# DeNA/Chainer_Realtime_Multi-Person_Pose_Estimation

Measured on AMD Instinct MI355X. Metric: frames/sec at 368x368 batch (1/2/4/8 GPU) + keypoint-match vs reference, higher is better.
Workload: dtype f32; 1 GPU; batch32_368x368_synthetic_uint8_per_gpu; per_gpu_batch=32, global_batch=32, map=320x320, weights=seeded He + calibrated head, records_gathered=32, status_bits=0

## Files before the change

### chainer_realtime_multi-person_pose_estimation_amd/csrc/conv_select.hip

```cpp
#include "pmx_common.h"

#include <math.h>
#include <algorithm>
#include <map>
#include <mutex>
#include <tuple>
#include <vector>

bool wino_eligible(int ks, int cin_pad, int cout_pad) { return (ks == 3 || ks == 7) && cin_pad % 32 == 0 && cout_pad % 128 == 0; }

static const double WINO_T7_CHUNK_US = 50.0, WINO_T3_CHUNK_US = 9.3, WINO_PHASE_US = 4.0, WINO_UNIT_FIXED_US = 8.0;

static double wino_tail_makespan(int ks, int nch, int g, long long nblk, int ncu)
{
    std::vector<double> unit_us;
    for (int c = 0; c < nch; c += g) unit_us.push_back(std::min(g, nch - c) * (ks == 7 ? 8.0 : 2.0) * WINO_PHASE_US + WINO_UNIT_FIXED_US);
    if (ks == 7) {
        unit_us.push_back(nch * 2.0 * WINO_PHASE_US + WINO_UNIT_FIXED_US);
        unit_us.push_back(nch * 2.0 * WINO_PHASE_US + WINO_UNIT_FIXED_US);
        unit_us.push_back(nch * 0.5 * WINO_PHASE_US + WINO_UNIT_FIXED_US);
    }
    std::vector<double> cu((size_t)ncu, 0.0);
    auto cmp = [](double a, double b) { return a > b; };
    double end = 0.0;
// ... 85 lines not shown
        const double cost = (double)main_rounds + (best + 10.0) / t_block;
        if (best_g && (o.wino_tail == 1 || cost < plain_cost)) { plain_cost = cost; tg = best_g; }
    }
    if (g) {
        const double t_block = nch * (ks == 7 ? 52e-6 : 18.5e-6);
        const double eff = o.wino_unit_eff / 100.0 * (ks == 7 ? 1.0 : 0.75);
        const long long ublocks = (long long)((H + 7) / 8) * ((W + 15) / 16) * images * nb;
        const double est_unit = (double)ublocks / (ncu * eff) +
                                (double)ublocks * (S + 1) * 65536.0 / 3.0e12 / t_block + 0.03;
        if (est_unit < plain_cost && ublocks * S * 2 >= ncu) { *unit_g = gu; return 2; }
    }
    if (blocks * 100 >= (long long)o.wino_min_fill * rounds * ncu) { *run = geom_run; *tail_g = tg; return 1; }
    return 0;
}

int wino_split_images(const WinoSelectOpts& o, int ks, int cin_pad, int cout_pad, int cout, int ldc, int B, int groups, int H, int W, int pool)
{
    if (!o.wino_split || B < 2 || o.conv_algo != 1) return 0;
    int ug = 0, run = 0, tg = 0;
    if (wino_select(o, ks, cin_pad, cout_pad, cout, ldc, B * groups, H, W, pool, &ug, &run, &tg) != 1) return 0;
    const int nch = cin_pad / 32;
    const long long ncu = o.ncu, nb = cout_pad / 128;
    const long long rects = (long long)((H + 7) / 8) * ((W + 15) / 16);
    long long bpi;
    if (run) {
        const int ntiles = PMX_WINO_RUN_TX * ((H + 1) / 2), nblk = (ntiles + PMX_WINO_RUN_TILES - 1) / PMX_WINO_RUN_TILES, nfull = ntiles / PMX_WINO_RUN_TILES;
        bpi = (long long)(tg ? nfull : nblk) * (W / (PMX_WINO_RUN_TX * 2)) * nb * groups;
    } else
        bpi = rects * nb * groups;
    const long long total = bpi * B, full = total / ncu;
// ... 22 lines not shown
```

### chainer_realtime_multi-person_pose_estimation_amd/csrc/pmx_api.hip

```cpp
#include "pmx_ctx.h"

#include <math.h>
#include <stdarg.h>
#include <stdio.h>
#include <string.h>
#include <algorithm>
#include <functional>
#include <map>

static thread_local char g_err[1024] = "";
void pmx_set_error(const char* fmt, ...)
{
    va_list ap;
    va_start(ap, fmt);
    vsnprintf(g_err, sizeof(g_err), fmt, ap);
    va_end(ap);
}
extern "C" const char* pmx_last_error(void) { return g_err; }
extern "C" const char* pmx_version(void) { return "pose_mi355x 0.1 (gfx950, fp32 MFMA)"; }

extern "C" int pmx_device_count(int* n)
{
    PMX_CHECK(n, PMX_ERR_INVALID, "pmx_device_count: null");
    int c = 0;
// ... 259 lines not shown
    }
    return PMX_OK;
}

extern "C" int pmx_synchronize(pmx_ctx* c)
{
    PMX_CHECK(c, PMX_ERR_INVALID, "null ctx");
    PMX_DEV(c);
    PMX_HIP(hipStreamSynchronize(c->stream));
    return PMX_OK;
}

extern "C" int pmx_set_option(pmx_ctx* c, const char* key, int value)
{
    PMX_CHECK(c && key, PMX_ERR_INVALID, "null arg");
    if (!strcmp(key, "force_variant_k7")) c->opt_force[7] = value;
    else if (!strcmp(key, "force_variant_k3")) c->opt_force[3] = value;
    else if (!strcmp(key, "force_variant_k1")) c->opt_force[1] = value;
    else if (!strcmp(key, "keep_smoothed")) c->opt_keep_smoothed = value;
    else if (!strcmp(key, "stop_stage")) c->opt_stop_stage = value;
    else if (!strcmp(key, "kernel_gen")) c->opt_kernel_gen = value;
    else if (!strcmp(key, "fuse_pairs")) c->opt_fuse_pairs = value;
    else if (!strcmp(key, "fuse_conv1")) c->opt_fuse_conv1 = value;
    else if (!strcmp(key, "conv1_wino")) c->opt_conv1_wino = value;
    else if (!strcmp(key, "precise_lanes")) c->opt_precise_lanes = value < 1 ? 1 : (value > PMX_PR_LANES ? PMX_PR_LANES : value);
    else if (!strcmp(key, "precise_plain")) c->opt_precise_plain = value;
    else if (!strcmp(key, "precise_lane_priority")) c->opt_precise_lane_priority = value != 0;
    else if (!strcmp(key, "precise_table_cap")) c->opt_precise_table_cap = value < 1 ? 1 : value;
    else if (!strcmp(key, "cubic_rows")) c->opt_cubic_rows = value;
    else if (!strcmp(key, "precision")) {
// ... 5 lines not shown
    }
    else if (!strcmp(key, "f16_bn")) {
        PMX_CHECK(value == 0 || value == 64 || value == 128, PMX_ERR_INVALID,
                  "pmx_set_option: \"f16_bn\" = %d: 0 (the launch-size rule), 64 or 128 output channels per block", value);
        c->opt_f16_bn = value;
    }
    else if (!strcmp(key, "conv_algo")) c->opt_conv_algo = value;
    else if (!strcmp(key, "wino_min_fill")) c->opt_wino_min_fill = value;
    else if (!strcmp(key, "wino_unit_eff")) c->opt_wino_unit_eff = value;
    else if (!strcmp(key, "wino_geom")) c->opt_wino_geom = value;
    else if (!strcmp(key, "wino_tail")) c->opt_wino_tail = value;
    else if (!strcmp(key, "wino_tail_g")) c->opt_wino_tail_g = value;
    else if (!strcmp(key, "wino_unit_g")) c->opt_wino_unit_g = value;
    else if (!strcmp(key, "wino_split")) c->opt_wino_split = value;
    else if (!strcmp(key, "wino_tail_merge")) c->opt_wino_tail_merge = value;
    else if (!strcmp(key, "ksplit")) c->opt_ksplit = value;
    else if (!strcmp(key, "ksplit_plan")) c->opt_ksplit = value > 0 ? -value : 0;
    else if (!strcmp(key, "conv_min_lds")) c->opt_conv_min_lds = value;
    else if (!strcmp(key, "conv_v5_lds")) c->opt_conv_v5_lds = value;
    else if (!strcmp(key, "pp_generic")) c->opt_pp_generic = value;
    else if (!strcmp(key, "pp_limbs_slices")) c->opt_limbs_slices = value;
    else if (!strcmp(key, "peaks_gpu_branch")) { c->opt_gpu_branch_peaks = value; c->tab_in_h = -1; }
    else if (!strcmp(key, "kp_flip_x")) c->opt_kp_flip_x = value != 0;
    else if (!strcmp(key, "wgrad_strips")) c->opt_wgrad_strips = value;
    else if (!strcmp(key, "trunk_keep_g")) c->opt_trunk_keep_g = value != 0;
    else { pmx_set_error("pmx_set_option: unknown key '%s'", key); return PMX_ERR_INVALID; }
    return PMX_OK;
}

extern "C" int pmx_set_layer(pmx_ctx* c, const char* name, const float* w, const float* bias, int cout, int cin, int ks)
// ... 42 lines not shown
    DevBuf<T> d;
    int rc;
    if ((rc = d.alloc(j.total))) return rc;
    j.dst = d.get();
    if ((rc = pmx_pack_launch_one(kind, j, st))) return rc;
    PMX_HIP(hipStreamSynchronize(st));
    slot = std::move(d);
    return PMX_OK;
}
static int ensure_wino_pack(hipStream_t st, PackedLayer& L) { return derive_on_device(st, L, PMX_PACK_WINO, L.d_ww, pmx_pack_job_wino(L, nullptr)); }
static int ensure_conv1_pack(hipStream_t st, PackedLayer& L) { return derive_on_device(st, L, PMX_PACK_CONV1, L.d_ww, pmx_pack_job_conv1(L, nullptr)); }
static int ensure_bf16x3_pack(hipStream_t st, PackedLayer& L) { return derive_on_device(st, L, PMX_PACK_BF16X3, L.d_w3, pmx_pack_job_bf16x3(L, nullptr)); }
static int ensure_f16_pack(hipStream_t st, PackedLayer& L) { return derive_on_device(st, L, PMX_PACK_F16, L.d_w16, pmx_pack_job_f16(L, nullptr)); }

static const int SK_ZERO_BIAS = PMX_SK_ZERO_BIAS;
static int sk_reserve(pmx_ctx* c, const FwdCall& k, size_t need)
{
    int rc;
    if ((rc = k.ws.sk_scratch.ensure(need, k.stream))) return rc;
    if (!c->sk_zero_bias) {
        if ((rc = c->sk_zero_bias.alloc(SK_ZERO_BIAS))) return rc;
        PMX_HIP(hipMemsetAsync(c->sk_zero_bias, 0, SK_ZERO_BIAS * sizeof(float), k.stream));
    }
    return PMX_OK;
}
template <typename Reduce>
static int slab_redirect(pmx_ctx* c, const FwdCall& k, const ConvArgs& a0, int groups, int S, size_t slab, unsigned long long kbounds, ConvArgs& a, Reduce& r)
{
    PMX_CHECK(a0.cout_pad <= SK_ZERO_BIAS, PMX_ERR_INVALID, "split-K: cout_pad %d too large", a0.cout_pad);
    if (int rc = sk_reserve(c, k, slab * S * groups)) return rc;
    memset(&r, 0, sizeof r);
    for (int g = 0; g < groups; ++g) {
        float* base = k.ws.sk_scratch + (size_t)g * S * slab;
        r.slabs[g] = base; r.bias[g] = a0.g[g].bias; r.out[g] = a0.g[g].out; r.cout[g] = a0.g[g].cout;
        a.g[g].out = base; a.g[g].bias = c->sk_zero_bias; a.g[g].cout = a0.cout_pad;
    }
    a.ldc = a0.cout_pad; a.relu = 0; a.pool = 0; a.ksplit = S; a.slab_stride = (long long)slab; a.kbounds = kbounds;
    r.slab_stride = (long long)slab; r.B = a0.B; r.H = a0.H; r.W = a0.W; r.ld_slab = a0.cout_pad; r.ldc = a0.ldc;
    r.relu = a0.relu; r.pool = a0.pool;
    return PMX_OK;
}
static int launch_conv(pmx_ctx* c, const FwdCall& k, const ConvArgs& a0, int groups, int v, const SplitPlan& plan)
{
    ConvArgs a = a0;
    if (plan.S <= 1) {
        a.ksplit = 1; a.slab_stride = 0;
        return conv_launch(v, a, groups, c->opt_conv_min_lds, c->opt_conv_v5_lds, k.stream);
    }
    SplitKReduceArgs r;
    int rc = slab_redirect(c, k, a0, groups, plan.S, (size_t)a0.B * a0.H * a0.W * a0.cout_pad, plan.bounds, a, r);
// ... 180 lines not shown
{
    const ConvProf* pf = p.prof ? &p.pf : nullptr;
    if (p.form == FORM_WINO_RUN) return launch_wino_run(c, k, p.a, p.ks, p.groups, p.tail_g, pf);
    int rc;
    if (pf && (rc = prof_begin(c, k, pf->label(), pf->flops, pf->bytes, pf->issued))) return rc;
    switch (p.form) {
    case FORM_F16: rc = conv_f16_launch(p.ks, p.a, p.groups, c->opt_f16_bn, c->num_cus, k.stream); break;
    case FORM_WINO_UNITS: rc = launch_wino_units(c, k, p.a, p.ks, p.groups, p.unit_g); break;
    case FORM_WINO: rc = conv_wino_launch(p.a, p.ks, p.groups, k.stream); break;
    default: rc = launch_conv(c, k, p.a, p.groups, p.variant, p.split); break;
    }
    if (rc) return rc;
    return pf ? prof_end(c, k) : PMX_OK;
}

static int run_conv(pmx_ctx* c, const FwdCall& k, const char* label, PackedLayer* L0, PackedLayer* L1, const float* in0, const float* in1, int lda,
                    float* out0, float* out1, int ldc, int B, int H, int W, int relu, int pool, int level = -1, const char* half = nullptr)
{
    const bool seg = k.seg && level >= 0;
    int rc;
    if (!seg && !half && c->opt_wino_split && B >= 2 && L0->ks > 1 && c->opt_precision != 2 && wino_layers_ok(L0, L1)) {
        const int n0 = wino_split_images(wino_opts(c, k, L0->ks, L1 ? 2 : 1, lda), L0->ks, L0->cin_pad, L0->cout_pad, L0->cout, ldc, B, L1 ? 2 : 1, H, W, pool);
        if (n0 > 0 && n0 < B) {
            const size_t pin = (size_t)n0 * H * W * lda, pout = (size_t)n0 * (pool ? H / 2 : H) * (pool ? W / 2 : W) * ldc;
            const std::string h0 = "@0+" + std::to_string(n0), h1 = "@" + std::to_string(n0) + "+" + std::to_string(B - n0);
            if ((rc = run_conv(c, k, label, L0, L1, in0, in1, lda, out0, out1, ldc, n0, H, W, relu, pool, level, h0.c_str()))) return rc;
            return run_conv(c, k, label, L0, L1, in0 + pin, in1 ? in1 + pin : nullptr, lda, out0 + pout, out1 ? out1 + pout : nullptr, ldc, B - n0, H, W, relu, pool, level,
                            h1.c_str());
        }
    }
    ConvPlan p;
    if ((rc = plan_conv(c, k, p, label, L0, L1, in0, in1, lda, out0, out1, ldc, B, H, W, relu, pool, level))) return rc;
    if (half && p.prof) p.pf.suffix = half;
    return launch_plan(c, k, p);
}

static int run_pair(pmx_ctx* c, const FwdCall& k, const char* labelA, const char* labelB, PackedLayer* a0, PackedLayer* a1, PackedLayer* b0, PackedLayer* b1,
                    const float* in0, const float* in1, int lda, float* mid0, float* mid1, int ldm, float* out0, float* out1, int ldc, int B,
                    int H, int W, int reluB, int level = -1, bool keep_mid = false)
{
    const PackedLayer& LA = *a0;
    const PackedLayer& LB = *b0;
    const int groups = a1 ? 2 : 1;
    const bool seg = k.seg && level >= 0;
    const long long npix = seg ? k.seg->pix[level] : (long long)B * H * W;
    const bool ok = !keep_mid && c->opt_fuse_pairs && c->opt_kernel_gen >= 6 && LA.ks == 1 && LB.ks == 1 && LA.cin_pad == 128 && LB.cin == LA.cout &&
                    conv_pair_supported(LA.cin, LA.cout, LB.cout_pad) && (groups == 1 || b1->cout_pad == LB.cout_pad);
    int rc;
    PMX_CHECK(ok || !seg, PMX_ERR_INVALID, "heterogeneous forward: the 1x1 pair %s + %s has no fused form", labelA, labelB);
    if (!ok) {
        if ((rc = run_conv(c, k, labelA, a0, a1, in0, in1, lda, mid0, mid1, ldm, B, H, W, 1, 0))) return rc;
        return run_conv(c, k, labelB, b0, b1, mid0, mid1, ldm, out0, out1, ldc, B, H, W, reluB, 0);
    }
    PairArgs p;
    memset(&p, 0, sizeof p);
    double flops = 0;
    for (int g = 0; g < groups; ++g) {
        const PackedLayer& A = *(g ? a1 : a0);
        const PackedLayer& Bl = *(g ? b1 : b0);
        p.g[g].in = g ? in1 : in0; p.g[g].w1 = A.d_w; p.g[g].b1 = A.d_b; p.g[g].w2 = Bl.d_w; p.g[g].b2 = Bl.d_b;
        p.g[g].out = g ? out1 : out0; p.g[g].cout = Bl.cout;
        flops += 2.0 * (double)npix * ((double)A.cout * A.cin + (double)Bl.cout * Bl.cin);
    }
    p.npix = npix; p.lda = lda; p.ldc = ldc; p.cmid = LA.cout; p.cout_pad = LB.cout_pad; p.relu2 = reluB;
    if (c->prof_on == 1) {
        const std::string kn = "conv1x1_pair_c" + std::to_string(LA.cout) + "_n" + std::to_string(LB.cout_pad);
        if ((rc = prof_begin(c, k, std::string(labelA) + "+" + labelB + "|" + kn, flops, 4.0 * (double)npix * groups * (LA.cin + LB.cout)))) return rc;
    }
    if ((rc = conv_pair_launch(p, groups, k.stream))) return rc;
    return prof_end(c, k);
}

static bool conv1_pairable(const pmx_ctx* c)
{
    const PackedLayer& L1 = c->layers[c->index.at("conv1_1")];
    const PackedLayer& L2 = c->layers[c->index.at("conv1_2")];
    return c->opt_precision == 0 && c->opt_force[3] < 0 && L1.cin == 3 && L1.cout == 64 && L2.cin == 64 && L2.cout == 64;
}
static bool trunk_retaining(const pmx_ctx* c, const FwdCall& k)
{
    return c->bw.on == 2 && c->kind == NET_POSE && c->ls_on && c->lg_on && c->opt_precision == 0 && !k.seg;
}
static bool conv1_form(const pmx_ctx* c, const FwdCall& k, int B, int H, int W, bool* fuse_out)
// ... 27 lines not shown
    if (seg && c->opt_precision == 2) {
        PMX_CHECK(!in_u8, PMX_ERR_STATE, "conv1: a uint8 input in f16 mode");
        if ((rc = run_conv(c, k, "conv1_1", &L1, nullptr, ws.in16, nullptr, PMX_IN_C, ws.act0, nullptr, 64, B, H, W, 1, 0, 0))) return rc;
        return run_conv(c, k, "conv1_2", &L2, nullptr, ws.act0, nullptr, 64, ws.act1, nullptr, 64, B, H, W, 1, 1, 0);
    }
    PMX_CHECK(!seg || (wino1 && in_u8), PMX_ERR_INVALID, "heterogeneous forward: needs conv1 as conv1_wino_kernel on a uint8 input");
    if (!fuse && !wino1) {
        if ((rc = run_conv(c, k, "conv1_1", &L1, nullptr, ws.in16, nullptr, PMX_IN_C, ws.act0, nullptr, 64, B, H, W, 1, 0))) return rc;
        return run_conv(c, k, "conv1_2", &L2, nullptr, ws.act0, nullptr, 64, ws.act1, nullptr, 64, B, H, W, 1, 1);
    }
    ConvArgs a;
    memset(&a, 0, sizeof a);
    a.g[0].in = ws.in16; a.g[0].w = L2.d_w; a.g[0].bias = L2.d_b; a.g[0].out = ws.act1; a.g[0].cout = L2.cout;
    a.g[1].w = L1.d_w; a.g[1].bias = L1.d_b;
    a.B = B; a.H = H; a.W = W; a.lda = PMX_IN_C; a.ldc = 64; a.nch = L2.nch; a.cout_pad = L2.cout_pad; a.relu = 1; a.pool = 1;
    if (wino1) {
        if ((rc = ensure_wino_pack(k.stream, L2)) || (rc = ensure_conv1_pack(k.stream, L1))) return rc;
        a.g[0].w = L2.d_ww;
        a.g[1].w = L1.d_ww;
        if (in_u8) {
            a.g[1].in = reinterpret_cast<const float*>(in_u8);
            a.kbounds = (unsigned long long)__builtin_bit_cast(unsigned, k.in_div);
        }
        if (seg) { a.nseg = (int)k.seg->segs.size(); a.segs = k.seg->table(PMX_SEG_CONV1); a.seg_tiles = k.seg->tiles[PMX_SEG_CONV1]; }
        if (c->prof_on == 1) {
            const double np0 = seg ? (double)k.seg->pix[0] : (double)B * H * W;
            const double f1 = 2.0 * np0 * 9.0 * (double)L1.cout * L1.cin, f2 = 2.0 * np0 * 9.0 * (double)L2.cout * L2.cin;
            if ((rc = prof_begin(c, k, "conv1_1+conv1_2|conv_wino1_f2x2_t16x16", f1 + f2, (in_u8 ? 3.0 : 4.0 * 3) * np0 + 4.0 * np0 * (64 / 4), f1 + f2 * 16.0 / 36.0))) return rc;
        }
        if ((rc = conv1_wino_launch(a, k.stream))) return rc;
// ... 94 lines not shown
}

int pmx_forward_from_in16(pmx_ctx* c, const FwdCall& k, int B, int H, int W)
{
    PMX_CHECK(!k.seg || c->kind == NET_POSE, PMX_ERR_INVALID, "heterogeneous forward: posenet only");
    if (c->kind != NET_POSE) return forward_cpm(c, k, B, H, W);
    NetBufs& ws = k.ws;
    auto L = [&](const char* n) { return &c->layers[c->index.at(n)]; };
    int rc;
    const int H8 = H / 8, W8 = W / 8;
#define RUN(...) do { if ((rc = run_conv(c, k, __VA_ARGS__))) return rc; } while (0)
    const bool hook = c->ls_on && !k.seg;
    PMX_CHECK(!hook || (&ws == static_cast<NetBufs*>(c) && k.stream == c->stream), PMX_ERR_STATE, "forward: the validation-loss hook covers the context's own working set only");
    BwState& bw = c->bw;
    const bool keep = bw.on && hook && c->lg_on && c->opt_precision == 0;
    bw.valid = bw.done = bw.trunk_done = false;
    const long long npix8 = (long long)B * H8 * W8;
    PMX_CHECK(!keep || (size_t)npix8 <= bw.cap_px, PMX_ERR_CAPACITY, "forward: %lld map pixels, the backward store holds %zu", npix8, bw.cap_px);
    auto slot = [&](int sl, float* else_) { return keep ? bw.act + bw.slot[sl].a_off : else_; };
    float* const x42 = slot(PMX_BW_X42, ws.act1);
    float* const a43 = slot(PMX_BW_C43, ws.act0);
    auto keep_stage = [&](int sl) {
        return keep ? bwd_copy_cols_launch(ws.cat + PMX_CAT_PAF, PMX_CAT_C, bw.act + bw.slot[sl].a_off, 64, npix8, 64, k.stream) : PMX_OK;
    };
    if ((rc = keep && bw.on == 2 ? run_stem_retaining(c, k, B, H, W, x42) : run_stem(c, k, B, H, W, keep ? x42 : nullptr))) return rc;
    RUN("conv4_3_CPM", L("conv4_3_CPM"), nullptr, x42, nullptr, 512, a43, nullptr, 256, B, H8, W8, 1, 0, 3);
    RUN("conv4_4_CPM", L("conv4_4_CPM"), nullptr, a43, nullptr, 256, ws.cat + PMX_CAT_FEAT, nullptr, PMX_CAT_C, B, H8, W8, 1, 0, 3);
    float* cat = ws.cat;
    float* const s51 = slot(PMX_BW_S1 + 0, ws.brA);
    float* const s52 = slot(PMX_BW_S1 + 1, ws.brB);
// ... 21 lines not shown
            in = o;
        }
        snprintf(n1, sizeof n1, "Mconv6_stage%d_L1", s); snprintf(n2, sizeof n2, "Mconv6_stage%d_L2", s);
        snprintf(m1, sizeof m1, "Mconv7_stage%d_L1", s); snprintf(m2, sizeof m2, "Mconv7_stage%d_L2", s);
        snprintf(lab, sizeof lab, "Mconv6_stage%d", s); snprintf(lab2, sizeof lab2, "Mconv7_stage%d", s);
        float* const m6 = slot(PMX_BW_M(s, 6), ws.brB);
        if ((rc = run_pair(c, k, lab, lab2, L(n1), L(n2), L(m1), L(m2), in, in + 128, 256, m6, m6 + 128, 256,
                           cat + PMX_CAT_PAF, cat + PMX_CAT_HEAT, PMX_CAT_C, B, H8, W8, 0, 3, keep))) return rc;
        n_stages = s;
        if (hook && (rc = pmx_loss_stage(c, s, B, H8, W8))) return rc;
        if ((rc = keep_stage(PMX_BW_M(s, 7)))) return rc;
    }
    if (hook && (rc = pmx_loss_finish(c, n_stages, B, H8, W8))) return rc;
    if (keep) { bw.valid = true; bw.stages = n_stages; bw.B = B; bw.fh = H8; bw.fw = W8; bw.t_H = H; bw.t_W = W; }
#undef RUN
    c->maps_valid = true; c->maps_external = false;
    c->cur_B = B; c->cur_fh = H8; c->cur_fw = W8;
    c->cur_segs.clear();
    c->pp_valid = false;
    return PMX_OK;
}

int pmx_check_weights(pmx_ctx* c)
{
    int missing = 0;
    for (auto& l : c->layers) missing += l.set ? 0 : 1;
    PMX_CHECK(missing == 0, PMX_ERR_WEIGHTS, "forward: %d of %d layers have no weights", missing, (int)c->layers.size());
    return PMX_OK;
}
static int check_forward_args(pmx_ctx* c, const void* p, int B, int H, int W)
// ... 24 lines not shown
{
    int rc;
    if (k.seg && c->opt_precision == 2) {
        const long long np0 = k.seg->pix[0];
        PMX_CHECK(np0 >= 1 && np0 <= (long long)c->max_batch * c->max_h * c->max_w && np0 < (1ll << 31), PMX_ERR_CAPACITY,
                  "heterogeneous forward: %lld input pixels", np0);
        if (c->prof_on == 1 && (rc = prof_begin(c, k, "prep_u8|prep_u8", 0, (double)np0 * (3 + 64)))) return rc;
        if ((rc = launch_prep_u8(d, k.ws.in16, 1, 1, (int)np0, divisor, k.stream))) return rc;
        if ((rc = prof_end(c, k))) return rc;
        return pmx_forward_from_in16(c, k, B, H, W);
    }
    if (k.seg || conv1_form(c, k, B, H, W, nullptr)) {
        FwdCall ku = k;
        ku.in_u8 = d; ku.in_div = divisor;
        return pmx_forward_from_in16(c, ku, B, H, W);
    }
    if (c->prof_on == 1 && (rc = prof_begin(c, k, "prep_u8|prep_u8", 0, (double)B * H * W * (3 + 64)))) return rc;
    if ((rc = launch_prep_u8(d, k.ws.in16, B, H, W, divisor, k.stream))) return rc;
    if ((rc = prof_end(c, k))) return rc;
    return pmx_forward_from_in16(c, k, B, H, W);
}

extern "C" int pmx_forward_f32(pmx_ctx* c, const float* x, int B, int H, int W, int on_device)
{
    int rc = check_forward_args(c, x, B, H, W);
    if (rc) return rc;
    PMX_DEV(c);
    const float* d = x;
    if (!on_device) {
        PMX_HIP(hipMemcpyAsync(c->nchw_tmp, x, (size_t)B * H * W * 3 * sizeof(float), hipMemcpyHostToDevice, c->stream));
// ... 313 lines not shown
    PMX_HIP(hipStreamSynchronize(c->stream));
    c->pp_valid = false;
    return pp_realloc(c, cap_pk, cap_sub, candidates, cap_ppl);
}

extern "C" int pmx_get_capacities(pmx_ctx* c, int* peaks_per_joint, int* subsets, int* people, int* candidates)
{
    PMX_CHECK(c, PMX_ERR_INVALID, "null ctx");
    if (peaks_per_joint) *peaks_per_joint = c->pp.cap_pk;
    if (subsets) *subsets = c->pp.cap_sub;
    if (people) *people = c->pp.cap_ppl;
    if (candidates) *candidates = c->pp.cap_cand;
    return PMX_OK;
}

extern "C" int pmx_detect_batch(pmx_ctx* c, const uint8_t* img, int B, int H, int W, int on_device, int map_h, int map_w,
                                double img_len, const double* scale_xy)
{
    int rc = pmx_forward_u8(c, img, B, H, W, on_device);
    if (rc) return rc;
    return pmx_postprocess(c, B, map_h, map_w, img_len, scale_xy);
}

extern "C" int pmx_results_layout(pmx_ctx* c, int* people_cap, size_t* bytes_per_record)
{
    PMX_CHECK(c, PMX_ERR_INVALID, "null ctx");
    PMX_CHECK(c->pp_valid, PMX_ERR_STATE, "pmx_results_layout: no post-process results yet");
    PMX_DEV(c);
    int rc = pp_finalize(c);
    if (rc) return rc;
    if (people_cap) *people_cap = c->pp.cap_ppl;
    if (bytes_per_record) *bytes_per_record = c->pp.rec_bytes;
    return PMX_OK;
// ... 463 lines not shown
```

### chainer_realtime_multi-person_pose_estimation_amd/csrc/pmx_common.h

```cpp
#pragma once
#include <hip/hip_runtime.h>
#include <stdint.h>
#include <stddef.h>
#include <atomic>
#include <string>
#include <vector>

#include "../../include/pose_mi355x.h"
#include "pp_tables.h"

#define PMX_HEATMAP_PEAK_THRESH 0.05f
#define PMX_N_INTEG_POINTS 10
#define PMX_N_INTEG_POINTS_THRESH 8
#define PMX_INNER_PRODUCT_THRESH 0.05
#define PMX_LIMB_LENGTH_RATIO 1.0
#define PMX_LENGTH_PENALTY_VALUE 1.0
#define PMX_N_SUBSET_LIMBS_THRESH 3.0
#define PMX_SUBSET_SCORE_THRESH 0.2
#define PMX_GAUSS_SIGMA 2.5

static const int PMX_LIMBS[PMX_N_LIMBS][2] = {
    {1, 8}, {8, 9}, {9, 10}, {1, 11}, {11, 12}, {12, 13}, {1, 2}, {2, 3}, {3, 4}, {2, 16},
    {1, 5}, {5, 6}, {6, 7}, {5, 17}, {1, 0}, {0, 14}, {0, 15}, {14, 16}, {15, 17}};

// ... 86 lines not shown
int conv_wino_run_launch(const ConvArgs& a, int ks, int groups, hipStream_t stream, hipEvent_t e0 = nullptr, hipEvent_t e1 = nullptr);
int conv_wino_merged_tail_launch(const ConvArgs& a, int ks, int groups, hipStream_t stream);
struct WinoSelectOpts {
    int conv_algo, precision, forced_variant, ksplit, wino_unit_eff, wino_min_fill, wino_geom, wino_tail, wino_tail_g;
    int wino_tail_merge = 1;
    int wino_split = 1;
    int wino_unit_g = 0;
    int groups = 1;
    int lda = 0;
    int ncu;
};
bool wino_eligible(int ks, int cin_pad, int cout_pad);
int wino_select(const WinoSelectOpts& o, int ks, int cin_pad, int cout_pad, int cout, int ldc, int images, int H, int W, int pool, int* unit_g,
                int* run, int* tail_g);
int wino_split_images(const WinoSelectOpts& o, int ks, int cin_pad, int cout_pad, int cout, int ldc, int B, int groups, int H, int W, int pool);
struct SplitPlan { int S; unsigned long long bounds; int sizes[8]; };
struct SplitKReduceArgs {
    const float* slabs[2];
    const float* bias[2];
    float* out[2];
    int cout[2];
    long long slab_stride;
    int ksplit, B, H, W, ld_slab, ldc, relu, pool;
};
int conv_splitk_reduce(const SplitKReduceArgs& r, int groups, hipStream_t stream);
struct PairGroupArgs {
    const float* in;
    const float* w1; const float* b1;
    const float* w2; const float* b2;
    float* out;
// ... 88 lines not shown
```

### chainer_realtime_multi-person_pose_estimation_amd/csrc/pmx_ctx.h

```cpp
#pragma once
#include "pmx_common.h"
#include "pack_index.h"

#include <map>
#include <tuple>
#include <string>
#include <utility>
#include <vector>

template <typename T, bool Host = false>
struct DevBuf {
    T* p = nullptr;
    size_t cap = 0;
    DevBuf() = default;
    DevBuf(const DevBuf&) = delete;
    DevBuf& operator=(const DevBuf&) = delete;
    DevBuf(DevBuf&& o) noexcept { swap(o); }
    DevBuf& operator=(DevBuf&& o) noexcept { reset(); swap(o); return *this; }
    ~DevBuf() { reset(); }
    void swap(DevBuf& o) noexcept { std::swap(p, o.p); std::swap(cap, o.cap); }
    T* get() const { return p; }
    operator T*() const { return p; }
    size_t capacity() const { return cap; }
    void reset()
// ... 121 lines not shown
};

struct SegDesc { int n, H, W; };
enum { PMX_SEG_CONV1 = 0, PMX_SEG_L1 = 1, PMX_SEG_L1P = 2, PMX_SEG_L2 = 3, PMX_SEG_L2P = 4, PMX_SEG_L3 = 5, PMX_SEG_L0 = 6, PMX_SEG_L0P = 7,
       PMX_SEG_TABLES = 8 };
#define PMX_SEG_RECT(level, pool) ((level) == 0 ? ((pool) ? PMX_SEG_L0P : PMX_SEG_L0) : (level) == 1 ? ((pool) ? PMX_SEG_L1P : PMX_SEG_L1) \
                                   : (level) == 2 ? ((pool) ? PMX_SEG_L2P : PMX_SEG_L2) : PMX_SEG_L3)
struct SegGeo { int n, H, W, mh, mw; };
struct SegTables {
    std::vector<SegDesc> segs;
    int tiles[PMX_SEG_TABLES] = {};
    long long pix[4] = {};
    const ConvSeg* dev = nullptr;
    const ConvSeg* table(int t) const { return dev + (size_t)t * segs.size(); }
};
struct FwdCall {
    NetBufs& ws;
    hipStream_t stream;
    int conv_algo;
    const SegTables* seg = nullptr;
    const uint8_t* in_u8 = nullptr;
    float in_div = 255.0f;
};
struct PPCall { PPMaps maps; PPTables tab; int base, B, map_h, map_w; double img_len; bool has_scale; int limbs_slices; };

enum { PMX_BW_C43 = 0, PMX_BW_C44 = 1, PMX_BW_S1 = 2, PMX_BW_M2 = 7, PMX_BW_X42 = 42, PMX_BW_SLOTS = 43 };
#define PMX_BW_M(s, i) (PMX_BW_M2 + ((s) - 2) * 7 + (i) - 1)
struct BwSlot { size_t a_off = 0, g_off = 0; int lda = 0, ldg = 0; };
struct BwState {
    int on = 0;
    bool valid = false;
    bool done = false;
    int stages = 0, B = 0, fh = 0, fw = 0;
    size_t cap_px = 0;
    BwSlot slot[PMX_BW_SLOTS];
    DevBuf<float> act, g;
    DevBuf<float> grad;
// ... 97 lines not shown
    int opt_force[8] = {-1, -1, -1, -1, -1, -1, -1, -1};
    int opt_gpu_branch_peaks = 0;
    int opt_limbs_slices = -1;
    int pp_limbs_slices = 0;
    int opt_kp_flip_x = 0;
    int tab_flip = 0;
    int opt_keep_smoothed = 0, opt_stop_stage = 6, opt_kernel_gen = 6;
    int opt_conv_algo = 1;
    int opt_wino_unit_eff = 80;
    int opt_wino_min_fill = 50;
    int opt_wino_geom = -1;
    int opt_wino_tail = -1;
    int opt_wino_tail_merge = 1;
    int opt_wino_tail_g = 0;
    int opt_wino_split = 1;
    int opt_wino_unit_g = 0;
    int opt_precision = 0;
    int opt_f16_bn = 0;
    int opt_conv1_wino = 1;
    int opt_fuse_conv1 = 1;
    int opt_fuse_pairs = 1;
    int opt_ksplit = 0;
    int opt_conv_min_lds = 0;
    int opt_conv_v5_lds = 56 * 1024;
    int opt_pp_generic = 0;
    int opt_cubic_rows = 1;
    DevBuf<float> sk_zero_bias;
    Event t0, t1;
    int prof_on = 0;
    std::vector<ProfEntry> prof;
// ... 100 lines not shown
```

Baseline: 954.8 frames/s.

## Split batch into two concurrent image chains on separate streams

Adds a batch-chains mode that splits the batch in half and runs the whole forward pass and postprocessing for each half on its own HIP stream, with per-chain split-K scratch buffers. A probe pass checks whether every layer can be split cleanly by images and whether the 7x7 Winograd block counts divide evenly into CU rounds. In automatic mode the split is used only when those checks pass. The intent is to fill the GPU during each layer's tail by overlapping the two chains, at the cost of a probe pass, extra launches and possible contention between the streams.

```diff
diff --git a/chainer_realtime_multi-person_pose_estimation_amd/csrc/conv_select.hip b/chainer_realtime_multi-person_pose_estimation_amd/csrc/conv_select.hip
--- a/chainer_realtime_multi-person_pose_estimation_amd/csrc/conv_select.hip
+++ b/chainer_realtime_multi-person_pose_estimation_amd/csrc/conv_select.hip
@@ -123,6 +123,19 @@
     return 0;
 }
 
+bool batch_chains_rounds(const WinoSelectOpts& o, int mode, int run, int tail_g, int cout_pad, int n0, int n1, int H, int W)
+{
+    if (mode != 1 || o.conv_algo != 1 || o.precision != 0) return false;
+    const long long nb = cout_pad / 128, grp = std::max(1, o.groups);
+    long long bpi;
+    if (run) {
+        const int ntiles = PMX_WINO_RUN_TX * ((H + 1) / 2), nblk = (ntiles + PMX_WINO_RUN_TILES - 1) / PMX_WINO_RUN_TILES, nfull = ntiles / PMX_WINO_RUN_TILES;
+        bpi = (long long)(tail_g ? nfull : nblk) * (W / (PMX_WINO_RUN_TX * 2)) * nb * grp;
+    } else
+        bpi = (long long)((H + 7) / 8) * ((W + 15) / 16) * nb * grp;
+    return n0 >= 1 && n1 >= 1 && bpi * n0 % o.ncu == 0 && bpi * n1 % o.ncu == 0;
+}
+
 int wino_split_images(const WinoSelectOpts& o, int ks, int cin_pad, int cout_pad, int cout, int ldc, int B, int groups, int H, int W, int pool)
 {
     if (!o.wino_split || B < 2 || o.conv_algo != 1) return 0;
diff --git a/chainer_realtime_multi-person_pose_estimation_amd/csrc/pmx_api.hip b/chainer_realtime_multi-person_pose_estimation_amd/csrc/pmx_api.hip
--- a/chainer_realtime_multi-person_pose_estimation_amd/csrc/pmx_api.hip
+++ b/chainer_realtime_multi-person_pose_estimation_amd/csrc/pmx_api.hip
@@ -297,6 +297,7 @@
 extern "C" int pmx_set_option(pmx_ctx* c, const char* key, int value)
 {
     PMX_CHECK(c && key, PMX_ERR_INVALID, "null arg");
+    c->opt_epoch += 1;
     if (!strcmp(key, "force_variant_k7")) c->opt_force[7] = value;
     else if (!strcmp(key, "force_variant_k3")) c->opt_force[3] = value;
     else if (!strcmp(key, "force_variant_k1")) c->opt_force[1] = value;
@@ -332,6 +333,10 @@
     else if (!strcmp(key, "wino_unit_g")) c->opt_wino_unit_g = value;
     else if (!strcmp(key, "wino_split")) c->opt_wino_split = value;
     else if (!strcmp(key, "wino_tail_merge")) c->opt_wino_tail_merge = value;
+    else if (!strcmp(key, "batch_chains")) {
+        PMX_CHECK(value >= -1 && value <= 1, PMX_ERR_INVALID, "pmx_set_option: \"batch_chains\" = %d: 0 (off), 1 (wherever the plans allow) or -1 (automatic)", value);
+        c->opt_batch_chains = value;
+    }
     else if (!strcmp(key, "ksplit")) c->opt_ksplit = value;
     else if (!strcmp(key, "ksplit_plan")) c->opt_ksplit = value > 0 ? -value : 0;
     else if (!strcmp(key, "conv_min_lds")) c->opt_conv_min_lds = value;
@@ -404,13 +409,16 @@
 static int ensure_f16_pack(hipStream_t st, PackedLayer& L) { return derive_on_device(st, L, PMX_PACK_F16, L.d_w16, pmx_pack_job_f16(L, nullptr)); }
 
 static const int SK_ZERO_BIAS = PMX_SK_ZERO_BIAS;
+static DevBuf<float>& sk_slabs(const FwdCall& k) { return k.scratch ? k.scratch->sk_scratch : k.ws.sk_scratch; }
+static DevBuf<float>& sk_zeros(pmx_ctx* c, const FwdCall& k) { return k.scratch ? k.scratch->sk_zero_bias : c->sk_zero_bias; }
 static int sk_reserve(pmx_ctx* c, const FwdCall& k, size_t need)
 {
     int rc;
-    if ((rc = k.ws.sk_scratch.ensure(need, k.stream))) return rc;
-    if (!c->sk_zero_bias) {
-        if ((rc = c->sk_zero_bias.alloc(SK_ZERO_BIAS))) return rc;
-        PMX_HIP(hipMemsetAsync(c->sk_zero_bias, 0, SK_ZERO_BIAS * sizeof(float), k.stream));
+    if ((rc = sk_slabs(k).ensure(need, k.stream))) return rc;
+    DevBuf<float>& zero = sk_zeros(c, k);
+    if (!zero) {
+        if ((rc = zero.alloc(SK_ZERO_BIAS))) return rc;
+        PMX_HIP(hipMemsetAsync(zero, 0, SK_ZERO_BIAS * sizeof(float), k.stream));
     }
     return PMX_OK;
 }
@@ -421,9 +429,9 @@
     if (int rc = sk_reserve(c, k, slab * S * groups)) return rc;
     memset(&r, 0, sizeof r);
     for (int g = 0; g < groups; ++g) {
-        float* base = k.ws.sk_scratch + (size_t)g * S * slab;
+        float* base = sk_slabs(k) + (size_t)g * S * slab;
         r.slabs[g] = base; r.bias[g] = a0.g[g].bias; r.out[g] = a0.g[g].out; r.cout[g] = a0.g[g].cout;
-        a.g[g].out = base; a.g[g].bias = c->sk_zero_bias; a.g[g].cout = a0.cout_pad;
+        a.g[g].out = base; a.g[g].bias = sk_zeros(c, k); a.g[g].cout = a0.cout_pad;
     }
     a.ldc = a0.cout_pad; a.relu = 0; a.pool = 0; a.ksplit = S; a.slab_stride = (long long)slab; a.kbounds = kbounds;
     r.slab_stride = (long long)slab; r.B = a0.B; r.H = a0.H; r.W = a0.W; r.ld_slab = a0.cout_pad; r.ldc = a0.ldc;
@@ -634,6 +642,53 @@
     return pf ? prof_end(c, k) : PMX_OK;
 }
 
+static FwdCall chain_call(const FwdCall& k, int i, int B, int* first, int* n)
+{
+    FwdCall kc = k;
+    kc.split = nullptr;
+    *first = i ? k.split->n0 : 0;
+    *n = i ? B - k.split->n0 : k.split->n0;
+    if (i) { kc.stream = k.split->second->stream; kc.scratch = k.split->second; }
+    return kc;
+}
+static std::string chain_suffix(int first, int n) { return "@" + std::to_string(first) + "+" + std::to_string(n); }
+static int launch_plan_chains(pmx_ctx* c, const FwdCall& k, const ConvPlan& p)
+{
+    ChainSplit& s = *k.split;
+    const ConvArgs& a = p.a;
+    if (s.probe) {
+        if (p.form == FORM_WINO_RUN && p.tail_g)
+            for (int n : {s.n0, a.B - s.n0}) {
+                ConvArgs h = a;
+                h.B = n;
+                if (wino_tail_merged(c, h) != wino_tail_merged(c, a)) s.ok = false;
+            }
+        if (p.ks == 7 && !batch_chains_rounds(wino_opts(c, k, p.ks, p.groups, a.lda), p.form == FORM_WINO || p.form == FORM_WINO_RUN, p.form == FORM_WINO_RUN,
+                                              p.tail_g, a.cout_pad, s.n0, a.B - s.n0, a.H, a.W)) s.rounds = false;
+        return PMX_OK;
+    }
+    const size_t pin = (size_t)a.H * a.W * a.lda, pout = (size_t)(a.pool ? a.H / 2 : a.H) * (a.pool ? a.W / 2 : a.W) * a.ldc;
+    auto second = [&](const float* ptr, size_t per_image) {
+        const NetBufs& ws = k.ws;
+        if (ptr >= ws.act0 && ptr < ws.act0 + ws.act0.capacity()) return (size_t)s.n0 * s.net_px * 64;
+        if (ptr >= ws.act1 && ptr < ws.act1 + ws.act1.capacity()) return (size_t)s.n0 * s.net_px * 16;
+        return (size_t)s.n0 * per_image;
+    };
+    for (int i = 0; i < 2; ++i) {
+        int first, n;
+        const FwdCall kc = chain_call(k, i, a.B, &first, &n);
+        ConvPlan q = p;
+        q.a.B = n;
+        for (int g = 0; g < p.groups && i; ++g) { q.a.g[g].in += second(a.g[g].in, pin); q.a.g[g].out += second(a.g[g].out, pout); }
+        if (q.prof) {
+            const double share = (double)n / a.B;
+            q.pf.flops *= share; q.pf.bytes *= share; q.pf.issued *= share; q.pf.suffix = chain_suffix(first, n);
+        }
+        if (int rc = launch_plan(c, kc, q)) return rc;
+    }
+    return PMX_OK;
+}
+
 static int run_conv(pmx_ctx* c, const FwdCall& k, const char* label, PackedLayer* L0, PackedLayer* L1, const float* in0, const float* in1, int lda,
                     float* out0, float* out1, int ldc, int B, int H, int W, int relu, int pool, int level = -1, const char* half = nullptr)
 {
@@ -641,6 +696,11 @@
     int rc;
     if (!seg && !half && c->opt_wino_split && B >= 2 && L0->ks > 1 && c->opt_precision != 2 && wino_layers_ok(L0, L1)) {
         const int n0 = wino_split_images(wino_opts(c, k, L0->ks, L1 ? 2 : 1, lda), L0->ks, L0->cin_pad, L0->cout_pad, L0->cout, ldc, B, L1 ? 2 : 1, H, W, pool);
+        if (n0 > 0 && n0 < B && k.split) {
+            PMX_CHECK(k.split->probe, PMX_ERR_STATE, "two chains: layer %s is cut in two by images", label ? label : "?");
+            k.split->ok = false;
+            return PMX_OK;
+        }
         if (n0 > 0 && n0 < B) {
             const size_t pin = (size_t)n0 * H * W * lda, pout = (size_t)n0 * (pool ? H / 2 : H) * (pool ? W / 2 : W) * ldc;
             const std::string h0 = "@0+" + std::to_string(n0), h1 = "@" + std::to_string(n0) + "+" + std::to_string(B - n0);
@@ -652,7 +712,7 @@
     ConvPlan p;
     if ((rc = plan_conv(c, k, p, label, L0, L1, in0, in1, lda, out0, out1, ldc, B, H, W, relu, pool, level))) return rc;
     if (half && p.prof) p.pf.suffix = half;
-    return launch_plan(c, k, p);
+    return k.split ? launch_plan_chains(c, k, p) : launch_plan(c, k, p);
 }
 
 static int run_pair(pmx_ctx* c, const FwdCall& k, const char* labelA, const char* labelB, PackedLayer* a0, PackedLayer* a1, PackedLayer* b0, PackedLayer* b1,
@@ -683,10 +743,23 @@
         flops += 2.0 * (double)npix * ((double)A.cout * A.cin + (double)Bl.cout * Bl.cin);
     }
     p.npix = npix; p.lda = lda; p.ldc = ldc; p.cmid = LA.cout; p.cout_pad = LB.cout_pad; p.relu2 = reluB;
-    if (c->prof_on == 1) {
-        const std::string kn = "conv1x1_pair_c" + std::to_string(LA.cout) + "_n" + std::to_string(LB.cout_pad);
-        if ((rc = prof_begin(c, k, std::string(labelA) + "+" + labelB + "|" + kn, flops, 4.0 * (double)npix * groups * (LA.cin + LB.cout)))) return rc;
-    }
+    const std::string name = std::string(labelA) + "+" + labelB + "|conv1x1_pair_c" + std::to_string(LA.cout) + "_n" + std::to_string(LB.cout_pad);
+    const double bytes = 4.0 * (double)npix * groups * (LA.cin + LB.cout);
+    if (k.split) {
+        if (k.split->probe) return PMX_OK;
+        for (int i = 0; i < 2; ++i) {
+            int first, n;
+            const FwdCall kc = chain_call(k, i, B, &first, &n);
+            PairArgs q = p;
+            q.npix = (long long)n * H * W;
+            for (int g = 0; g < groups; ++g) { q.g[g].in += (size_t)first * H * W * lda; q.g[g].out += (size_t)first * H * W * ldc; }
+            const double share = (double)n / B;
+            if (c->prof_on == 1 && (rc = prof_begin(c, kc, name + chain_suffix(first, n), flops * share, bytes * share))) return rc;
+            if ((rc = conv_pair_launch(q, groups, kc.stream)) || (rc = prof_end(c, kc))) return rc;
+        }
+        return PMX_OK;
+    }
+    if (c->prof_on == 1 && (rc = prof_begin(c, k, name, flops, bytes))) return rc;
     if ((rc = conv_pair_launch(p, groups, k.stream))) return rc;
     return prof_end(c, k);
 }
@@ -744,6 +817,30 @@
     a.g[0].in = ws.in16; a.g[0].w = L2.d_w; a.g[0].bias = L2.d_b; a.g[0].out = ws.act1; a.g[0].cout = L2.cout;
     a.g[1].w = L1.d_w; a.g[1].bias = L1.d_b;
     a.B = B; a.H = H; a.W = W; a.lda = PMX_IN_C; a.ldc = 64; a.nch = L2.nch; a.cout_pad = L2.cout_pad; a.relu = 1; a.pool = 1;
+    if (k.split) {
+        if (k.split->probe) return PMX_OK;
+        if (wino1 && ((rc = ensure_wino_pack(k.stream, L2)) || (rc = ensure_conv1_pack(k.stream, L1)))) return rc;
+        if (wino1) { a.g[0].w = L2.d_ww; a.g[1].w = L1.d_ww; }
+        if (wino1 && in_u8) a.kbounds = (unsigned long long)__builtin_bit_cast(unsigned, k.in_div);
+        const double f1 = 2.0 * H * W * 9.0 * (double)L1.cout * L1.cin, f2 = 2.0 * H * W * 9.0 * (double)L2.cout * L2.cin;
+        for (int i = 0; i < 2; ++i) {
+            int first, n;
+            const FwdCall kc = chain_call(k, i, B, &first, &n);
+            ConvArgs q = a;
+            q.B = n;
+            q.g[0].in += (size_t)first * H * W * PMX_IN_C; q.g[0].out += (size_t)first * (H / 2) * (W / 2) * 64;
+            if (wino1 && in_u8) q.g[1].in = reinterpret_cast<const float*>(in_u8 + (size_t)first * H * W * 3);
+            if (c->prof_on == 1) {
+                const double np = (double)n * H * W;
+                rc = wino1 ? prof_begin(c, kc, "conv1_1+conv1_2|conv_wino1_f2x2_t16x16" + chain_suffix(first, n), n * (f1 + f2),
+                                        (in_u8 ? 3.0 : 4.0 * 3) * np + 4.0 * np * (64 / 4), n * (f1 + f2 * 16.0 / 36.0))
+                           : prof_begin(c, kc, "conv1_1+conv1_2|conv1_fused_t8x16_n64" + chain_suffix(first, n), n * (f1 + f2), 4.0 * np * (3 + 64 / 4));
+                if (rc) return rc;
+            }
+            if ((rc = wino1 ? conv1_wino_launch(q, kc.stream) : conv1_fused_launch(q, kc.stream)) || (rc = prof_end(c, kc))) return rc;
+        }
+        return PMX_OK;
+    }
     if (wino1) {
         if ((rc = ensure_wino_pack(k.stream, L2)) || (rc = ensure_conv1_pack(k.stream, L1))) return rc;
         a.g[0].w = L2.d_ww;
@@ -868,6 +965,7 @@
     PMX_CHECK(!hook || (&ws == static_cast<NetBufs*>(c) && k.stream == c->stream), PMX_ERR_STATE, "forward: the validation-loss hook covers the context's own working set only");
     BwState& bw = c->bw;
     const bool keep = bw.on && hook && c->lg_on && c->opt_precision == 0;
+    PMX_CHECK(!k.split || !hook, PMX_ERR_STATE, "forward: two chains under the validation-loss hook");
     bw.valid = bw.done = bw.trunk_done = false;
     const long long npix8 = (long long)B * H8 * W8;
     PMX_CHECK(!keep || (size_t)npix8 <= bw.cap_px, PMX_ERR_CAPACITY, "forward: %lld map pixels, the backward store holds %zu", npix8, bw.cap_px);
@@ -919,6 +1017,7 @@
     if (hook && (rc = pmx_loss_finish(c, n_stages, B, H8, W8))) return rc;
     if (keep) { bw.valid = true; bw.stages = n_stages; bw.B = B; bw.fh = H8; bw.fw = W8; bw.t_H = H; bw.t_W = W; }
 #undef RUN
+    if (k.split && k.split->probe) return PMX_OK;
     c->maps_valid = true; c->maps_external = false;
     c->cur_B = B; c->cur_fh = H8; c->cur_fw = W8;
     c->cur_segs.clear();
@@ -973,6 +1072,16 @@
         FwdCall ku = k;
         ku.in_u8 = d; ku.in_div = divisor;
         return pmx_forward_from_in16(c, ku, B, H, W);
+    }
+    if (k.split) {
+        for (int i = 0; i < 2 && !k.split->probe; ++i) {
+            int first, n;
+            const FwdCall kc = chain_call(k, i, B, &first, &n);
+            if (c->prof_on == 1 && (rc = prof_begin(c, kc, "prep_u8|prep_u8" + chain_suffix(first, n), 0, (double)n * H * W * (3 + 64)))) return rc;
+            if ((rc = launch_prep_u8(d + (size_t)first * H * W * 3, k.ws.in16 + (size_t)first * H * W * PMX_IN_C, n, H, W, divisor, kc.stream))) return rc;
+            if ((rc = prof_end(c, kc))) return rc;
+        }
+        return pmx_forward_from_in16(c, k, B, H, W);
     }
     if (c->prof_on == 1 && (rc = prof_begin(c, k, "prep_u8|prep_u8", 0, (double)B * H * W * (3 + 64)))) return rc;
     if ((rc = launch_prep_u8(d, k.ws.in16, B, H, W, divisor, k.stream))) return rc;
@@ -1316,9 +1425,88 @@
     return PMX_OK;
 }
 
+static int chains_wanted(pmx_ctx* c, const uint8_t* d, int B, int H, int W, bool* yes)
+{
+    *yes = false;
+    if (!c->opt_batch_chains || B < 2 || c->kind != NET_POSE || c->opt_precision != 0 || c->ls_on || c->bw.on || c->tr.on || c->opt_keep_smoothed) return PMX_OK;
+    if (c->opt_batch_chains < 0 && (c->opt_conv_algo != 1 || c->prof_on == 1)) return PMX_OK;
+    const int key[4] = {B, H, W, c->opt_epoch};
+    if (memcmp(key, c->chains_key, sizeof key)) {
+        ChainSplit s;
+        s.n0 = B / 2; s.probe = true;
+        FwdCall k = pmx_call(c);
+        k.split = &s;
+        c->chains_key[3] = -1;
+        if (int rc = pmx_forward_from_u8(c, k, d, B, H, W, 255.0f)) return rc;
+        memcpy(c->chains_key, key, sizeof key);
+        c->chains_ok = s.ok; c->chains_rounds = s.rounds;
+    }
+    *yes = c->chains_ok && (c->opt_batch_chains > 0 || c->chains_rounds);
+    return PMX_OK;
+}
+
+static int detect_batch_chains(pmx_ctx* c, const uint8_t* d, int B, int H, int W, int map_h, int map_w, double img_len, const double* scale_xy)
+{
+    BatchChain& ch = c->chain2;
+    int rc;
+    if ((rc = ch.stream.create(hipStreamNonBlocking)) || (rc = ch.fork.create(hipEventDisableTiming)) || (rc = ch.done.create(hipEventDisableTiming))) return rc;
+    if ((rc = pmx_ensure_tables(c, H / 8, W / 8, map_h, map_w))) return rc;
+    const double* dscale = nullptr;
+    if (scale_xy) {
+        PMX_HIP(hipMemcpyAsync(c->d_scale, scale_xy, sizeof(double) * 2 * B, hipMemcpyHostToDevice, c->stream));
+        dscale = c->d_scale;
+    }
+    PMX_HIP(hipEventRecord(ch.fork, c->stream));
+    PMX_HIP(hipStreamWaitEvent(ch.stream, ch.fork, 0));
+    ChainSplit s;
+    s.n0 = B / 2; s.net_px = (size_t)H * W; s.second = &ch;
+    FwdCall k = pmx_call(c);
+    k.split = &s;
+    rc = pmx_forward_from_u8(c, k, d, B, H, W, 255.0f);
+    const PPMaps m = pmx_current_maps(c);
+    c->pp_limbs_slices = c->opt_limbs_slices >= 0 ? c->opt_limbs_slices : 0;
+    struct ProfCtx { pmx_ctx* c; FwdCall k; std::string suffix; };
+    auto prof_cb = [](void* v, const char* name, int begin) {
+        ProfCtx* p = (ProfCtx*)v;
+        if (begin) (void)prof_begin(p->c, p->k, std::string(name) + "|" + name + p->suffix, 0, 0);
+        else (void)prof_end(p->c, p->k);
+    };
+    for (int i = 0; i < 2 && !rc; ++i) {
+        int first, n;
+        ProfCtx pc{c, chain_call(k, i, B, &first, &n), ""};
+        pc.suffix = chain_suffix(first, n);
+        PPMaps mi = m;
+        mi.heat += first * m.sbh; mi.paf += first * m.sbp;
+        rc = pp_launch(mi, c->tab, pmx_pp_view(c->pp, first), n, map_h, map_w, img_len, dscale ? dscale + 2 * first : nullptr, 0, c->opt_pp_generic, pc.k.stream,
+                       c->prof_on == 1 ? +prof_cb : nullptr, &pc, c->pp_limbs_slices);
+    }
+    PMX_HIP(hipEventRecord(ch.done, ch.stream));
+    PMX_HIP(hipStreamWaitEvent(c->stream, ch.done, 0));
+    if (rc) return rc;
+    c->pp_valid = true; c->pp_final = false; c->pp_B = B; c->pp_h = map_h; c->pp_w = map_w;
+    c->pp_maps = m; c->pp_img_len = img_len; c->pp_has_scale = scale_xy != nullptr;
+    c->pp_calls.clear();
+    return PMX_OK;
+}
+
 extern "C" int pmx_detect_batch(pmx_ctx* c, const uint8_t* img, int B, int H, int W, int on_device, int map_h, int map_w,
                                 double img_len, const double* scale_xy)
 {
+    bool chains = false;
+    if (c && img && c->opt_batch_chains && map_h >= 1 && map_w >= 1 && (long long)map_h * map_w < (1ll << 31)) {
+        int rc = check_forward_args(c, img, B, H, W);
+        if (rc) return rc;
+        PMX_DEV(c);
+        if ((rc = chains_wanted(c, img, B, H, W, &chains))) return rc;
+        if (chains) {
+            const uint8_t* d = img;
+            if (!on_device) {
+                PMX_HIP(hipMemcpyAsync(c->u8_tmp, img, (size_t)B * H * W * 3, hipMemcpyHostToDevice, c->stream));
+                d = c->u8_tmp;
+            }
+            return detect_batch_chains(c, d, B, H, W, map_h, map_w, img_len, scale_xy);
+        }
+    }
     int rc = pmx_forward_u8(c, img, B, H, W, on_device);
     if (rc) return rc;
     return pmx_postprocess(c, B, map_h, map_w, img_len, scale_xy);
diff --git a/chainer_realtime_multi-person_pose_estimation_amd/csrc/pmx_common.h b/chainer_realtime_multi-person_pose_estimation_amd/csrc/pmx_common.h
--- a/chainer_realtime_multi-person_pose_estimation_amd/csrc/pmx_common.h
+++ b/chainer_realtime_multi-person_pose_estimation_amd/csrc/pmx_common.h
@@ -124,6 +124,7 @@
 int wino_select(const WinoSelectOpts& o, int ks, int cin_pad, int cout_pad, int cout, int ldc, int images, int H, int W, int pool, int* unit_g,
                 int* run, int* tail_g);
 int wino_split_images(const WinoSelectOpts& o, int ks, int cin_pad, int cout_pad, int cout, int ldc, int B, int groups, int H, int W, int pool);
+bool batch_chains_rounds(const WinoSelectOpts& o, int mode, int run, int tail_g, int cout_pad, int n0, int n1, int H, int W);
 struct SplitPlan { int S; unsigned long long bounds; int sizes[8]; };
 struct SplitKReduceArgs {
     const float* slabs[2];
diff --git a/chainer_realtime_multi-person_pose_estimation_amd/csrc/pmx_ctx.h b/chainer_realtime_multi-person_pose_estimation_amd/csrc/pmx_ctx.h
--- a/chainer_realtime_multi-person_pose_estimation_amd/csrc/pmx_ctx.h
+++ b/chainer_realtime_multi-person_pose_estimation_amd/csrc/pmx_ctx.h
@@ -159,6 +159,17 @@
     const ConvSeg* dev = nullptr;
     const ConvSeg* table(int t) const { return dev + (size_t)t * segs.size(); }
 };
+struct BatchChain {
+    Stream stream;
+    Event fork, done;
+    DevBuf<float> sk_scratch, sk_zero_bias;
+};
+struct ChainSplit {
+    int n0 = 0;
+    size_t net_px = 0;
+    BatchChain* second = nullptr;
+    bool probe = false, ok = true, rounds = true;
+};
 struct FwdCall {
     NetBufs& ws;
     hipStream_t stream;
@@ -166,6 +177,8 @@
     const SegTables* seg = nullptr;
     const uint8_t* in_u8 = nullptr;
     float in_div = 255.0f;
+    ChainSplit* split = nullptr;
+    BatchChain* scratch = nullptr;
 };
 struct PPCall { PPMaps maps; PPTables tab; int base, B, map_h, map_w; double img_len; bool has_scale; int limbs_slices; };
 
@@ -293,6 +306,11 @@
     int opt_wino_tail_merge = 1;
     int opt_wino_tail_g = 0;
     int opt_wino_split = 1;
+    int opt_batch_chains = -1;
+    BatchChain chain2;
+    int chains_key[4] = {0, 0, 0, -1};
+    bool chains_ok = false, chains_rounds = false;
+    int opt_epoch = 0;
     int opt_wino_unit_g = 0;
     int opt_precision = 0;
     int opt_f16_bn = 0;
```

Result: faster. 966.7 frames/s, median of 6 (+1.2%).
